# kikimo/tla-raft

Measured on AMD Instinct MI355X. Metric: distinct states/sec (whole node) + wall-time to exhaust, higher is better.
Workload: dtype u32

## Files before the change

tla-raft_amd/csrc/rmc_engine.hip:

```cpp
#include <hip/hip_runtime.h>
#include <hipcub/hipcub.hpp>

#include <algorithm>
#include <array>
#include <chrono>
#include <condition_variable>
#include <cstdio>
#include <cstdlib>
#include <cstring>
#include <memory>
#include <mutex>
#include <string>
#include <thread>
#include <vector>

#include <fcntl.h>
#include <sys/mman.h>
#include <unistd.h>

#include "rmc.h"
#include "rmc_kernels.h"
#include "rmc_plan.h"
#include "rmc_spec.h"

// ... 448 lines not shown
    std::vector<TraceStep> trace;
    double seconds = 0;

    KParams base(const Shard &s) const {
        KParams P{};
        P.d = U.d;
        P.E = cfg.max_election;
        P.R = cfg.max_restart;
        P.seeded = cfg.spec_variant == RMC_SPEC_SEEDED;
        P.quirks = (cfg.spec_variant == RMC_SPEC_SPLIT_BRAIN ? 1u : 0u) | (cfg.spec_variant == RMC_SPEC_COMMIT_PAST_LOG ? 2u : 0u);
        P.check_deadlock = cfg.check_deadlock;
        P.inv_mask = cfg.invariants;
        P.inv_order = inv_order;
        P.t.info = d_info;
        P.t.nat2id = d_nat2id;
        P.t.gmsg = d_gmsg;
        P.t.seeds = d_seeds;
        P.t.np = np;
        P.t.bmw = (uint32_t)((U.info.size() + 31) / 32);
        P.seen = s.seen();
        P.rcap = ~0ull;
        P.err = s.err;
        P.flags = s.flags;
        P.par = s.par;
        P.pslot = s.pslot;
        P.trace_base = s.tdev;
        return P;
    }

    void ring_params(const Shard &s, KParams &P) const {
        P.front = s.R;
        P.foff = s.cur_off;
        P.fbase = s.cur_wbase;
        P.rcap = s.rcap;
        P.next = s.R;
        P.noff = s.nxt_off;
        P.nbase = s.nbase();
    }

    KParams chunk_params(const Shard &s) const {
        KParams Q = base(s);
        ring_params(s, Q);
        Q.cnt = s.cnt; Q.fp = s.fp; Q.wpos = s.wpos; Q.wcnt = s.wcnt; Q.wacc = s.wacc; Q.pnm = s.pnm;
        Q.wposw = s.wposw; Q.bw = s.bw; Q.bg = s.bg; Q.boff = s.boff; Q.bww = s.bww; Q.boffw = s.boffw;
        Q.bn = s.bn; Q.boffn = s.boffn;
        Q.tickets = s.tickets; Q.ctick = s.ctick; Q.sum = s.sum;
        Q.score = s.score; Q.lslot = s.lslot; Q.ET = s.E; Q.hctx = s.hctx;
        return Q;
    }

    const int lookahead = env_int("RMC_LOOKAHEAD", 1, 0, 1);
    bool two_sets() const { return lookahead && !multi; }

    void swap_staging(Shard &s) {
        Staging &a = s.alt;
        std::swap(s.score, a.score); std::swap(s.hctx, a.hctx); std::swap(s.cnt, a.cnt); std::swap(s.pnm, a.pnm);
        std::swap(s.hcnt, a.hcnt); std::swap(s.hoff, a.hoff);
        std::swap(s.err, a.err); std::swap(s.sum, a.sum); std::swap(s.flags, a.flags);
        std::swap(s.xdone, a.done); std::swap(s.xt0, a.t0); std::swap(s.xt1, a.t1); std::swap(s.xtimed, a.timed);
        s.ocnt = reinterpret_cast<uint32_t *>(s.sum + SUM_OCNT);
    }
    static void alt_params(const Staging &a, KParams &Q) {
        Q.score = a.score; Q.hctx = a.hctx; Q.cnt = a.cnt; Q.pnm = a.pnm;
        Q.err = a.err; Q.sum = a.sum; Q.flags = a.flags;
    }
    void xwait() {
        if (xpending) HIPCHK(hipStreamSynchronize(xstream));
    }
    void drop_lookahead() {
        if (!xpending) return;
        xpending = false;
        (void)hipStreamSynchronize(xstream);
        Shard &s = sh[0];
        (void)hipMemsetAsync(s.alt.err, 0xFF, ERR_NSLOTS * 8, xstream);
        (void)hipMemsetAsync(s.alt.flags, 0, 16, xstream);
        (void)hipMemsetAsync(s.alt.sum, 0, SUM_WORDS_TOTAL * 8, xstream);
        (void)hipStreamSynchronize(xstream);
    }
    struct XDrain {
        rmc_ctx *c;
        ~XDrain() { c->drop_lookahead(); }
    };

    void pack(const int32_t *u, uint32_t *rec) const {
        const int n = N, Vv = V;
        std::vector<uint32_t> w(Layout<MAXN, MAXV>::NW + 8, 0);
        int k = 0;
        auto L_VF = 0, L_CT = 1, L_ROLE = 2, L_CI = 3, L_LL = 4, L_LOG = 5, L_MI = 5 + n, L_NI = 5 + 2 * n,
             L_PEND = 5 + 3 * n, L_MISC = 6 + 3 * n;
        auto check = [](int v, int lo, int hi, const char *what) {
            if (v < lo || v > hi) throw Fail(RMC_E_ARG, std::string("state field out of range: ") + what);
        };
        for (int i = 0; i < n; i++) {
            check(u[k + i], -1, n - 1, "votedFor");
            w[L_VF] = setnib(w[L_VF], i, u[k + i] < 0 ? VF_NONE : (uint32_t)u[k + i]);
        }
        k += n;
        for (int i = 0; i < n; i++) { check(u[k + i], 0, 7, "currentTerm"); w[L_CT] = setnib(w[L_CT], i, u[k + i]); }
        k += n;
        for (int i = 0; i < n; i++) { check(u[k + i], 0, 2, "role"); w[L_ROLE] = setnib(w[L_ROLE], i, u[k + i]); }
        k += n;
        for (int i = 0; i < n; i++) { check(u[k + i], 1, Vv + 1, "commitIndex"); w[L_CI] = setnib(w[L_CI], i, u[k + i]); }
        k += n;
        std::vector<int> ll(n);
        for (int i = 0; i < n; i++) {
            check(u[k + i], 1, Vv + 1, "Len(logs)");
// ... 1152 lines not shown
            for (Shard &t : sh) fix_ring(t, sh.size());
        replicated = false;
    }
    uint64_t *old_off_ = nullptr;
    int pending_fail = 0;
    std::string pending_msg;

    std::string flag_msg(unsigned long long f) const {
        if (f & 1u) return "a state exceeds msg_cap = " + std::to_string(ks.MCAP) + " messages";
        if (f & 2u) return "internal: a split chunk's parent records are not consecutive in the frontier ring";
        if (f & 4u) return "race probe: the commit's arrival counters were not all re-armed when the level finished";
        return "internal: unknown flag " + std::to_string(f);
    }
    static int flag_code(unsigned long long f) { return (f & 1u) ? RMC_E_CAPACITY : RMC_E_STATE; }

    static int first_error(const unsigned long long *e, unsigned long long *best) {
        int kind = -1;
        *best = ~0ull;
        const int order[4] = {ERR_ASSERT, ERR_DEADLOCK, ERR_INV, ERR_EVAL};
        for (int q = 0; q < 4; q++) {
            const int kk = order[q];
            if (e[kk] == ~0ull) continue;
            if (kind < 0 || (e[kk] >> 8) < (*best >> 8)) { kind = kk; *best = e[kk]; }
        }
        return kind;
    }

    void renew_election_tags(Shard &s, uint32_t ahead) {
        if (!s.E || s.epoch + ahead - s.lxy_epoch0 < 0xFFFFu) return;
        launch_eslot_clear(s.E, s.lcap, stream);
        s.lxy_epoch0 = s.epoch;
    }

    void end_level(Shard &s, uint64_t gid_nxt, int L) {
        std::swap(s.cur_off, s.nxt_off);
        std::swap(s.cur_off_cap, s.nxt_off_cap);
        s.cur_wbase = s.nbase();
        s.cur_words = s.nxt_words;
        s.nxt_words = 0;
        s.cur_n = s.nxt_n;
        s.nxt_n = 0;
        if (s.cur_n) s.level_start.push_back(gid_nxt);
        (void)L;
    }

    int step_single(rmc_level_stats *st) {
        auto t0 = std::chrono::steady_clock::now();
        Shard &s = sh[0];
        const int L = (int)s.level_start.size();
        st->level = L;
        st->expanded = s.cur_n;
        const uint64_t gid_cur = s.level_start[L - 1];
        const uint64_t gid_nxt = gid_cur + s.cur_n;
        uint64_t level_gen = 0, level_self = 0;
        s.nxt_n = 0;
        s.nxt_words = 0;
        const uint64_t MSW = (uint64_t)ks.maxsucc * (uint64_t)ks.RECW_MAX;
        XDrain drain{this};
        bool ahead = false;
        const bool time_hash = timing_on && (!cfg.timing_phases || (cfg.timing_phases & (1u << PH_HASH)));
        for (uint64_t p0 = 0; p0 < s.cur_n; p0 += chunk_parents) {
            const uint64_t p1 = std::min(s.cur_n, p0 + chunk_parents), np_ = p1 - p0;
            const bool expanded = ahead;
            ahead = false;
            if (expanded) {
                swap_staging(s);
                HIPCHK(hipStreamWaitEvent(stream, s.xdone, 0));
                xpending = false;
                if (s.xtimed) evrecs.push_back({PH_HASH, s.xt0, s.xt1});
            }
            const uint64_t Gub = np_ * (uint64_t)ks.maxsucc;
            maybe_migrate(s, s.T_count + Gub);
            const bool may_small = Gub <= (1ull << 20);
            uint64_t consumed = (s.ring_fixed && p0 && may_small) ? d2h(s.cur_off + p0) : 0;
            const bool small = may_small && seen_room(s, s.T_count + Gub) && ring_room(s, np_ * MSW, consumed);
            if (small) {
                ensure_ring(s, np_ * MSW, consumed);
                ensure_off(s.nxt_off, s.nxt_off_cap, s.nxt_n, s.nxt_n + Gub);
                grow_trace(s, Gub);
                grow_seen(s, s.T_count + Gub);
            }
            ensure_chunk(s, Gub);
            const uint64_t Lcap = std::min(next_pow2(2 * Gub), s.lcap);
            renew_election_tags(s, 1);
            ++s.epoch;
            trace_restart(s);
            const bool split = split_min && np_ >= split_min;
            const bool fold = split && ks.maxsucc <= 256;
            auto params = [&] {
                KParams Q = chunk_params(s);
                Q.p_begin = p0; Q.p_end = p1; Q.next_base = s.nxt_n; Q.next_wbase = s.nxt_words;
                Q.gid_next_base = gid_nxt; Q.gid_parent_base = gid_cur;
                Q.Lmask = Lcap - 1;
                Q.epoch = s.epoch;
                Q.split = split ? (fold ? 1 : 7) : 0;
                Q.plist = split ? s.plist : nullptr;
                Q.hcnt = split ? s.hcnt : nullptr;
                Q.hoff = fold ? s.hoff : nullptr;
                s.chunk_sep = Q.hcnt != nullptr;
                s.chunk_dense = Q.hoff != nullptr;
                return Q;
            };
            constexpr size_t SUM_CLEAR = (SUM_SELF_STRIPE + SELF_STRIDE * SELF_STRIPES - SUM_SELF) * 8;
            if (!expanded) {
                HIPCHK(hipMemsetAsync(s.sum + SUM_SELF, 0, SUM_CLEAR, stream));
                timed(PH_HASH, [&] {
                    if (split) ks.split(params(), stream);
                    else ks.fused(params(), stream);
                });
            }
            auto look_ahead = [&] {
                const uint64_t q1 = std::min(s.cur_n, p1 + chunk_parents);
                if (!two_sets() || !split || p1 >= s.cur_n || q1 - p1 < split_min || s.gslots < Gcap ||
                    !s.alt.score || !s.alt.hctx)
                    return;
                KParams Q = params();
                alt_params(s.alt, Q);
                Q.p_begin = p1;
                Q.p_end = q1;
                Q.hcnt = s.alt.hcnt;
                Q.hoff = fold ? s.alt.hoff : nullptr;
                xpending = true;
                HIPCHK(hipMemsetAsync(s.alt.sum + SUM_SELF, 0, SUM_CLEAR, xstream));
                s.alt.timed = time_hash;
                if (time_hash) HIPCHK(hipEventRecord(s.alt.t0, xstream));
                ks.split(Q, xstream);
                if (time_hash) HIPCHK(hipEventRecord(s.alt.t1, xstream));
                HIPCHK(hipEventRecord(s.alt.done, xstream));
                ahead = true;
            };
            look_ahead();
            if (split) timed(PH_OTHER, [&] { ks.hash_probe(params(), np_, stream); });
            timed(PH_DEDUP, [&] {
                ks.wincount(params(), np_, stream);
                if (split) launch_nzlist(params(), np_, stream);
            });
            if (!small) {
                HIPCHK(hipMemcpyAsync(s.hsum, s.sum, 8 * 8, hipMemcpyDeviceToHost, stream));
                unsigned long long *hc = s.hsum + SUM_WORDS_TOTAL - 1;
                const bool read_consumed = s.ring_fixed && p0 && !may_small;
                if (read_consumed) HIPCHK(hipMemcpyAsync(hc, s.cur_off + p0, 8, hipMemcpyDeviceToHost, stream));
                HIPCHK(hipStreamSynchronize(stream));
                if (read_consumed) consumed = *hc;
                collect_times(st);
                const uint64_t Wub = s.hsum[1], Wwords = s.hsum[SUM_WORDS];
                ensure_ring(s, Wwords, consumed);
                ensure_off(s.nxt_off, s.nxt_off_cap, s.nxt_n, s.nxt_n + Wub);
                grow_trace(s, Wub);
                grow_seen(s, s.T_count + Wub);
            }
            trace_fence(s);
            if (split && !fold) timed(PH_DEDUP, [&] { ks.insert(params(), np_, stream); });
            timed(PH_MAT, [&] {
                if (split) ks.commit_split(params(), np_, stream);
                else ks.commit(params(), stream);
            });
            HIPCHK(hipMemcpyAsync(s.hsum, s.sum, (SUM_SELF + 1) * 8, hipMemcpyDeviceToHost, stream));
            HIPCHK(hipStreamSynchronize(stream));
            HIPCHK(hipGetLastError());
            collect_times(st);
            const uint64_t G = s.hsum[0], Wn = s.hsum[1], Ww = s.hsum[SUM_WORDS];
            level_self += s.hsum[SUM_SELF];
            if (s.hsum[2 + ERR_NSLOTS]) throw Fail(flag_code(s.hsum[2 + ERR_NSLOTS]), flag_msg(s.hsum[2 + ERR_NSLOTS]));
            flush_trace(s, gid_nxt + s.nxt_n + Wn);
            level_gen += G;
            s.T_count += Wn;
            unsigned long long best;
            const int kind = first_error(s.hsum + 2, &best);
            if (kind >= 0) {
                drop_lookahead();
                stop_on_error(kind, best, p0, s.nxt_n, gid_cur, gid_nxt, level_gen - G, st);
                st->seconds = std::chrono::duration<double>(std::chrono::steady_clock::now() - t0).count();
                seconds += st->seconds;
                return status;
            }
            s.nxt_n += Wn;
            s.nxt_words += Ww;
            s.peak_words = std::max(s.peak_words, s.cur_words - consumed + s.nxt_words);
        }
        total_generated += level_gen;
        total_distinct += s.nxt_n;
        st->generated = level_gen;
        st->self_loops = level_self;
        st->new_states = s.nxt_n;
        st->new_bytes = s.nxt_words * 4;
        end_level(s, gid_nxt, L);
        if (s.cur_n) {
            depth = L + 1;
        } else {
            finished = true;
            status = RMC_DONE;
            queue_at_end = 0;
        }
        HIPCHK(hipStreamSynchronize(stream));
        st->total_generated = total_generated;
        st->total_distinct = total_distinct;
        st->queue = s.cur_n;
        st->status = finished ? RMC_DONE : RMC_OK;
        st->seconds = std::chrono::duration<double>(std::chrono::steady_clock::now() - t0).count();
        seconds += st->seconds;
        return st->status;
    }

    static int env_int(const char *name, int dflt, int lo, int hi) {
        const char *v = std::getenv(name);
        if (!v || !*v) return dflt;
        return std::max(lo, std::min(hi, std::atoi(v)));
    }
    const uint64_t split_min = (uint64_t)env_int("RMC_SPLIT_MIN", 1 << 16, 0, 1 << 30);
    const int dl_group = env_int("RMC_DL_GROUP", 2, 1, 64);
    const int dl_ahead = env_int("RMC_DL_AHEAD", 2, 1, 64);
    const int dl_query_us = env_int("RMC_DL_QUERY_US", 2000, 0, 1 << 30);
    int batch_levels() const { return cfg.device_levels ? (int)cfg.device_levels : LREC_CAP; }
    uint64_t dev_parents() const { return std::min<uint64_t>(chunk_parents, 1ull << 15); }
    bool batch_ok() const {
        const Shard &s = sh[0];
        const uint64_t first = s.cur_n * (uint64_t)ks.maxsucc;
        return (!multi || (replicated && s.cur_n < shard_min)) && inited && !finished && cfg.device_levels != 1 &&
               s.cur_n > 0 && s.cur_n <= dev_parents() && ring_room(s, first * (uint64_t)ks.RECW_MAX, 0) &&
               seen_room(s, s.T_count + 2 * first);
    }

    int step_batch(rmc_level_stats *out, int maxl) {
        auto t0 = std::chrono::steady_clock::now();
        Shard &s = sh[0];
        const uint64_t DP = dev_parents(), MS = (uint64_t)ks.maxsucc;
        const int K = std::max(1, std::min(maxl, LREC_CAP));
        uint64_t target = std::min(std::max<uint64_t>(s.cur_n * MS * 32, 1ull << 16), DP * MS);
        maybe_migrate(s, s.T_count + 2 * target);
        if (!ring_room(s, s.cur_n * MS * (uint64_t)ks.RECW_MAX, 0) || !seen_room(s, s.T_count + 2 * s.cur_n * MS))
            return 0;
        if (s.ring_fixed) target = std::min<uint64_t>(target, (s.rcap - s.cur_words) / (uint64_t)ks.RECW_MAX);
        if (s.Tc) target = std::min<uint64_t>(target, ((uint64_t)(0.9 * (double)s.T_cap) - s.T_count) / 2);
        target = std::max<uint64_t>(target, s.cur_n * MS);
        s.nxt_words = 0;
        ensure_ring(s, target * (uint64_t)ks.RECW_MAX, 0);
// ... 1632 lines not shown
```

tla-raft_amd/csrc/rmc_kernels.h:

```cpp
#pragma once
#include <hip/hip_runtime.h>
#include <stdint.h>

#include "rmc_spec.h"

namespace rmc {

struct Tables {
    const uint32_t *info;
    const uint16_t *nat2id;
    const ulonglong2 *gmsg;
    const uint64_t *seeds;
    int np;
    uint32_t bmw;
};

struct ESlot {
    unsigned long long x, y;
    unsigned long long k;
    unsigned long long pad;
};

struct Seen {
    ulonglong2 *T;
    unsigned long long *Tc;
    uint64_t mask;
    uint64_t cap;
};

enum ErrSlot { ERR_ASSERT = 0, ERR_DEADLOCK = 1, ERR_INV = 2, ERR_EVAL = 3, ERR_NSLOTS = 4 };

enum CtlStop : uint32_t { CTL_RUN = 0, CTL_DONE = 1, CTL_ERROR = 2, CTL_HOST = 3 };
struct LevelCtl {
    unsigned long long cur_n;
    unsigned long long gid_cur;
    unsigned long long T_count;
    unsigned long long Lmask;
    unsigned long long cur_wbase, cur_words;
    unsigned long long off_cap, rcap, trace_base, trace_cap, T_cap, chunk_parents, Lcap_max;
    uint32_t level;
    uint32_t epoch;
    uint32_t stop;
    uint32_t done_levels;
    uint32_t batch;
    uint32_t pad_;
};
struct LevelRec { unsigned long long expanded, generated, new_states, words, self_loops; };
constexpr int LREC_CAP = 1024;
struct HostLoop {
    uint32_t done;
    uint32_t stop;
    uint32_t pad_[2];
    LevelCtl ctl;
    LevelRec rec[LREC_CAP];
};
constexpr uint32_t WTILE = 1024;
constexpr uint32_t WTILES_MAX = 4096;
constexpr int SUM_WORDS = 7;
constexpr int SUM_INS = 9;
constexpr int SUM_INS_COMMIT = 10;
constexpr int SUM_NZ = 16;
constexpr int SUM_SELF = 17;
constexpr int SUM_HFP = 18;
constexpr int SUM_OCNT = 20;
constexpr int SUM_SELF_STRIPE = 64, SELF_STRIDE = 16, SELF_STRIPES = 8;
constexpr int SUM_WORDS_TOTAL = 192;


struct KParams {
    Dims d;
    int E, R, seeded, check_deadlock;
    uint32_t inv_mask;
    uint32_t inv_order;
    Tables t;
    const uint32_t *front;
    const uint64_t *foff;
    uint64_t fbase, rcap;
    uint64_t p_begin, p_end;
    uint32_t *cnt;
    uint32_t *hcnt;
    uint32_t *hoff;
    const uint32_t *off;
    ulonglong2 *fp;
    const uint32_t *wflag;
    uint32_t *wpos;
    Seen seen;
    uint32_t *next;
    uint64_t *noff;
    uint64_t nbase;
    uint64_t next_wbase;
    uint64_t next_base;
    uint64_t *par;
    uint16_t *pslot;
    uint64_t trace_base;
    uint64_t gid_next_base;
    uint64_t gid_parent_base;
    unsigned long long *err;
    uint32_t *flags;
    int route;
    uint4 *xside;
    uint32_t *ocnt;
    uint32_t nown;
    ESlot *OT;
    uint64_t ot_mask, gblk;
    uint32_t ot_round, self;
    int split;
    uint32_t *hctx;
    uint32_t quirks;
    uint4 *score;
    uint32_t *lslot;
    ESlot *ET;
    uint64_t Lmask;
    uint32_t epoch;
    uint32_t *wcnt;
    uint32_t *wacc;
    uint32_t *pnm;
    uint32_t *wposw;
    uint32_t *bw, *bg, *boff;
    uint32_t *bww, *boffw;
    uint32_t *bn, *boffn;
    uint32_t *plist;
    uint32_t *tickets;
    uint32_t *ctick;
    unsigned long long *sum;
    LevelCtl *ctl;
    LevelCtl *ctl_next;
    LevelRec *lrec;
    HostLoop *hloop;
    uint32_t done_levels;
    uint32_t *out_keys;
    uint32_t *out_count;
};

struct KernelSet {
    int N, V, MR, MCAP, CCW, RECW_MAX, maxsucc;
    int ctxw;
    void (*single)(const KParams &, hipStream_t);
    void (*fused)(const KParams &, hipStream_t);
    void (*split)(const KParams &, hipStream_t);
    void (*hash_probe)(const KParams &, uint64_t np, hipStream_t);
    void (*insert)(const KParams &, uint64_t np, hipStream_t);
    void (*wincount)(const KParams &, uint64_t np, hipStream_t);
    void (*commit)(const KParams &, hipStream_t);
    void (*commit_split)(const KParams &, uint64_t np, hipStream_t);
    void (*local_elect)(const KParams &, uint64_t np, Seen, ESlot *OT, uint64_t mask,
                        uint32_t round, uint32_t W, uint32_t self, uint64_t g0, hipStream_t);
    void (*local_flags)(const KParams &, uint64_t np, Seen, const ESlot *OT, uint32_t round, uint32_t W,
                        uint32_t self, uint64_t g0, unsigned long long *inserted, hipStream_t);
    void (*fp_states)(const KParams &, uint64_t n, hipStream_t);
    void (*inv_states)(const KParams &, uint64_t n, int32_t *out, hipStream_t);
    void (*encode)(const uint32_t *nibble_core, uint32_t *packed);
    void (*decode)(const uint32_t *packed, uint32_t *nibble_core);
};

bool get_kernels(int N, int V, int msg_cap, bool become_follower, KernelSet *ks);

constexpr uint32_t LS_SEEN = 0xFFFFFFFFu, LS_ELECT = 0xFFFFFFFEu, LS_WIN = 0xFFFFFFFDu;
void launch_rehash(const ulonglong2 *Told, uint64_t old_cap, Seen dst, hipStream_t s);
void launch_eslot_clear(ESlot *t, uint64_t n, hipStream_t s);
void launch_insert_fps(const ulonglong2 *fp, uint64_t n, Seen seen, hipStream_t s);
// ... 26 lines not shown
```

tla-raft_amd/csrc/rmc_kernels.hip:

```cpp
#include <hip/hip_runtime.h>


#include "rmc_kernels.h"

#ifdef RMC_PHASE_PROF
__device__ unsigned long long g_phase[16];
#define PHASE_DECL unsigned long long _acc[8] = {0, 0, 0, 0, 0, 0, 0, 0}; long long _tp = clock64();
#define PHASE(k) do { const long long _t = clock64(); _acc[k] += (unsigned long long)(_t - _tp); _tp = _t; } while (0)
#define PHASE_FLUSH_AT(b) do { if (threadIdx.x == 0) for (int _k = 0; _k < 8; _k++) atomicAdd(&g_phase[(b) + _k], _acc[_k]); } while (0)
#define PHASE_FLUSH PHASE_FLUSH_AT(0)
extern "C" int rmc_debug_phases(unsigned long long *out, int reset) {
    if (hipMemcpyFromSymbol(out, HIP_SYMBOL(g_phase), sizeof(unsigned long long) * 16) != hipSuccess) return -1;
    if (reset) {
        unsigned long long z[16] = {0};
        if (hipMemcpyToSymbol(HIP_SYMBOL(g_phase), z, sizeof(z)) != hipSuccess) return -1;
    }
    return 16;
}
#else
#define PHASE_DECL
#define PHASE(k) do {} while (0)
#define PHASE_FLUSH do {} while (0)
#define PHASE_FLUSH_AT(b) do {} while (0)
#endif
// ... 1029 lines not shown
    e[0] = a0.x; e[1] = a0.y; e[2] = a1.x; e[3] = a1.y; e[4] = a2.x; e[5] = a2.y; e[6] = a3.x; e[7] = a3.y;
}

__device__ __forceinline__ bool seen_contains(const Seen &S, ulonglong2 f) {
    if (S.Tc) {
        const uint64_t nbk = S.cap / TB;
        uint64_t b = t_home_c(f, nbk);
        for (;;) {
            unsigned long long e[TB];
            bucket_load(S.Tc, b, e);
            bool hit = false, free_ = false;
#pragma unroll
            for (uint64_t k = 0; k < TB; k++) {
                hit |= e[k] == f.x;
                free_ |= e[k] == 0ull;
            }
            if (hit) return true;
            if (free_) return false;
            b = (b + 1 == nbk) ? 0 : b + 1;
        }
    }
    uint64_t h = t_index(f, S.mask);
    for (;;) {
        const ulonglong2 e = S.T[h];
        asm volatile("" ::"v"(e.x), "v"(e.y));
        if (e.x == 0ull) return false;
        if (e.x == f.x && e.y == f.y) return true;
        h = (h + 1) & S.mask;
    }
}

__device__ __forceinline__ void seen_insert(const Seen &S, ulonglong2 f) {
    if (S.Tc) {
        const uint64_t nbk = S.cap / TB;
        uint64_t b = t_home_c(f, nbk);
        for (;;) {
            unsigned long long e[TB];
            bucket_load(S.Tc, b, e);
            for (uint64_t k = 0; k < TB; k++)
                if (e[k] == 0ull && atomicCAS(&S.Tc[b * TB + k], 0ull, (unsigned long long)f.x) == 0ull) return;
            b = (b + 1 == nbk) ? 0 : b + 1;
        }
    }
    uint64_t h = t_index(f, S.mask);
    for (;;) {
        unsigned long long prev = atomicCAS((unsigned long long *)&S.T[h].x, 0ull, (unsigned long long)f.x);
        if (prev == 0ull) { S.T[h].y = f.y; return; }
        h = (h + 1) & S.mask;
    }
}

__device__ __forceinline__ uint64_t l_index(const ulonglong2 f, uint64_t mask) {
    return (f.x ^ (f.x >> 31) ^ (f.y >> 7)) & mask;
}
__device__ __forceinline__ uint32_t fp_owner(const ulonglong2 f, uint32_t W) {
    return (uint32_t)((f.y >> 40) % W);
}

__device__ __forceinline__ uint32_t elect_tag(uint32_t epoch) { return epoch % 0xFFFFu + 1u; }
__device__ __forceinline__ unsigned long long elect_key(uint32_t epoch, uint64_t q, uint32_t e) {
    return ((unsigned long long)(0xFFFFFFFFu - epoch) << 32) | ((unsigned long long)(uint32_t)q << 2) | e;
}
__device__ __forceinline__ uint32_t elect_q(unsigned long long w) { return (uint32_t)w >> 2; }

template <int MAXS>
__device__ __forceinline__ uint32_t elect_slot(ESlot *E, uint32_t *wacc, uint64_t mask,
                                               uint32_t epoch, const ulonglong2 f, uint64_t q, uint32_t e, uint64_t g,
                                               unsigned long long v) {
    const unsigned long long tag = elect_tag(epoch);
    const unsigned long long xk = (f.x & ~0xFFFFull) | tag, yk = (f.y & ~0xFFFFull) | tag;
    for (;;) {
        unsigned long long *px = &E[g].x, *py = &E[g].y;
        if ((v & 0xFFFFull) != tag) {
            const unsigned long long prev = atomicCAS(px, v, xk);
            if (prev == v) {
#ifdef RMC_RACE_PROBE
                if ((q & 7u) == 0u) race_delay(2);
#endif
                __hip_atomic_store(py, yk, __ATOMIC_RELAXED, __HIP_MEMORY_SCOPE_AGENT);
                break;
            }
            v = prev;
            if ((v & 0xFFFFull) != tag) continue;
        }
        if (v == xk) {
            const unsigned long long y = __hip_atomic_load(py, __ATOMIC_RELAXED, __HIP_MEMORY_SCOPE_AGENT);
            if ((y & 0xFFFFull) != tag) {
                v = __hip_atomic_load(px, __ATOMIC_RELAXED, __HIP_MEMORY_SCOPE_AGENT);
                continue;
            }
            if (y == yk) break;
        }
        g = (g + 1) & mask;
        v = __hip_atomic_load(&E[g].x, __ATOMIC_RELAXED, __HIP_MEMORY_SCOPE_AGENT);
    }
    const unsigned long long mine = elect_key(epoch, q, e);
    const unsigned long long old = atomicMin(&E[g].k, mine);
    if (old > mine) {
        atomicAdd(&wacc[q / MAXS], 1u + (e << 12));
        if ((old >> 32) == (mine >> 32)) atomicSub(&wacc[elect_q(old) / MAXS], 1u + ((uint32_t)(old & 3u) << 12));
    }
    return (uint32_t)g;
}

template <int N, int V, int MR>
__device__ __forceinline__ void stage_succ(const Succ<N, V, MR> &o, uint32_t nm, uint4 *dst) {
// ... 991 lines not shown
            }
            if (tid < IC_N) sCc[tid] = 0u;
            __syncthreads();
            PHASE(6);
            if ((uint32_t)tid < nI) {
                const uint32_t kb = (sItm[j] - ibase) * NCI, cn = sCnt[j];
                const uint64_t pl = b0 + j;
                const uint64_t q0 = (!FUSE && P.hoff) ? (uint64_t)sHo[j] : pl * (uint64_t)MX;
#pragma unroll
                for (int c = 0; c < NCI; c++) {
                    const RowSucc<S::NADD> &x = c ? ob : o;
                    if (x.key == KEY_NONE || (!FUSE && x.self && P.hcnt)) continue;
                    uint32_t rank = 0;
                    for (uint32_t e = 0; e < cn; e++) rank += (uint32_t)sKey[kb + e] < x.key ? 1u : 0u;
                    const uint64_t q = q0 + rank;
                    if constexpr (FUSE) {
                        if (x.self) {
                            P.lslot[q] = LS_SEEN;
                            atomicAdd(&sSelfN, 1u);
                            continue;
                        }
                        uint4 st4[S::SW4];
                        row_stage<S::NADD>(x, nmj, S::SW4, st4);
                        uint4 *dst = P.score + q * (uint64_t)S::SW4;
#pragma unroll
                        for (int w = 0; w < S::SW4; w++) dst[w] = st4[w];
                        const unsigned long long *m0 = sM0 + j * NPR, *m1 = sM1 + j * NPR;
                        const ulonglong2 f = staged_fp<N, V, MR>(
                            P, sCore + j * NWP, [&](int pi) { return make_ulonglong2(m0[pi], m1[pi]); },
                            [&](int a, uint32_t) { return x.ainf[a]; }, st4[0], st4[1],
                            S::SW4 > 2 ? st4[S::SW4 > 2 ? 2 : 0] : make_uint4(0u, 0u, 0u, 0u), sK);
                        P.fp[q] = f;
                        P.lslot[q] = probe_elect<MX>(P, f, q, (x.nadd + (nmj & 1u) + 1u) >> 1, P.Lmask);
                    } else {
                        row_stage<S::NADD>(x, nmj, S::SW4, P.score + q * (uint64_t)S::SW4);
                    }
                }
            }
            PHASE(5);
            a = b;
        }
    }
    __syncthreads();
    if constexpr (FUSE) {
        if (tid == 0 && sSelfN)
            atomicAdd(&P.sum[SUM_SELF_STRIPE + SELF_STRIDE * (blockIdx.x % SELF_STRIPES)], (unsigned long long)sSelfN);
    } else {
        if (tid == 0 && sHfp) atomicAdd(&P.sum[SUM_HFP], (unsigned long long)sHfp);
    }
    PHASE_FLUSH;
}

template <int MX, class F>
__device__ __forceinline__ void each_successor(const KParams &P, F &&f) {
    const int lane = threadIdx.x & 63;
    const uint64_t np = P.p_end - P.p_begin;
    const uint64_t nwaves = (uint64_t)gridDim.x * (blockDim.x >> 6);
    for (uint64_t g0 = ((uint64_t)blockIdx.x * (blockDim.x >> 6) + (threadIdx.x >> 6)) * 64; g0 < np;
         g0 += nwaves * 64) {
        const uint64_t pl = g0 + (uint64_t)lane;
        const uint32_t t = pl < np ? (P.hcnt ? P.hcnt : P.cnt)[pl] : 0u;
        const uint32_t h0 = (pl < np && P.hoff) ? P.hoff[pl] : 0u;
        uint32_t tot;
        const uint32_t ex = wave_excl_scan(t, lane, &tot);
        for (uint32_t b0 = 0; b0 < tot; b0 += 64) {
            const uint32_t i = b0 + (uint32_t)lane;
            int j = 0;
#pragma unroll
            for (int st = 32; st; st >>= 1) {
                const uint32_t v = (uint32_t)__shfl(ex, j + st, 64);
                j = v <= i ? j + st : j;
            }
            const uint32_t exj = (uint32_t)__shfl(ex, j, 64);
            const uint32_t hj = (uint32_t)__shfl(h0, j, 64);
            const uint64_t pj = g0 + (uint64_t)j;
            if (i < tot) f(pj, i - exj, P.hoff ? (uint64_t)hj + (i - exj) : pj * (uint64_t)MX + (i - exj));
        }
    }
}

__device__ __forceinline__ unsigned long long owner_key(uint32_t tag, uint64_t key) {
    return ((unsigned long long)(0xFFFFu - tag) << 48) | key;
}
__device__ __forceinline__ uint64_t owner_order(uint64_t gparent, uint32_t rank, uint32_t e) {
    return (((gparent << 10) | rank) << 2) | e;
}
__device__ __forceinline__ bool owner_same(unsigned long long k, unsigned long long want) { return (k | 3ull) == (want | 3ull); }
struct OwnerLocal {
    uint32_t *wacc;
    uint64_t g0, np;
};
__device__ __forceinline__ uint32_t owner_bid(ESlot *OT, uint64_t mask, uint32_t tag32,
                                              const ulonglong2 f, uint64_t key, const OwnerLocal &loc) {
    const unsigned long long tag = tag32;
    const unsigned long long xk = (f.x & ~0xFFFFull) | tag, yk = (f.y & ~0xFFFFull) | tag;
    uint64_t g = l_index(f, mask);
    unsigned long long v = __hip_atomic_load(&OT[g].x, __ATOMIC_RELAXED, __HIP_MEMORY_SCOPE_AGENT);
    bool done = false;
    while (!done) {
        bool next = false;
        if ((v & 0xFFFFull) != tag) {
            const unsigned long long prev = atomicCAS(&OT[g].x, v, xk);
            if (prev == v) {
#ifdef RMC_RACE_PROBE
                if ((key & 7u) == 0u) race_delay(2);
#endif
                __hip_atomic_store(&OT[g].y, yk, __ATOMIC_RELAXED, __HIP_MEMORY_SCOPE_AGENT);
                done = true;
            } else {
                v = prev;
            }
        }
        if (!done && (v & 0xFFFFull) == tag) {
            if (v == xk) {
                const unsigned long long y = __hip_atomic_load(&OT[g].y, __ATOMIC_RELAXED, __HIP_MEMORY_SCOPE_AGENT);
                if (y == yk) done = true;
                else if ((y & 0xFFFFull) == tag) next = true;
                else v = __hip_atomic_load(&OT[g].x, __ATOMIC_RELAXED, __HIP_MEMORY_SCOPE_AGENT);
            } else {
                next = true;
            }
        }
        if (next) {
            g = (g + 1) & mask;
            v = __hip_atomic_load(&OT[g].x, __ATOMIC_RELAXED, __HIP_MEMORY_SCOPE_AGENT);
        }
    }
    const unsigned long long nk = owner_key(tag32, key);
    const unsigned long long old = atomicMin(&OT[g].k, nk);
    if (loc.wacc && nk < old) {
        const uint64_t gp = key >> 12;
        if (gp - loc.g0 < loc.np) atomicAdd(&loc.wacc[gp - loc.g0], 1u + ((uint32_t)(key & 3u) << 12));
        if ((old >> 48) == (unsigned long long)(0xFFFFu - tag32)) {
            const uint64_t ok = old & ((1ull << 48) - 1ull), op = ok >> 12;
            if (op - loc.g0 < loc.np) atomicSub(&loc.wacc[op - loc.g0], 1u + ((uint32_t)(ok & 3u) << 12));
        }
    }
    return (uint32_t)g;
}

#ifndef RMC_PROBE_WAVES
#define RMC_PROBE_WAVES 0
#endif
template <int N, int V, int MR, int MX>
__global__ __launch_bounds__(256, RMC_PROBE_WAVES) void k_hash_probe(KParams P) {
    using S = Spec<N, V, MR>;
    using Lo = Layout<N, V>;
    constexpr int CTXW = ctx_words<N, V>(), CC4 = (S::CCW + 3) / 4;
    __shared__ uint64_t sK[2][N * N];
    __shared__ uint32_t sOwn[64];
    if (threadIdx.x < 2 * N * N) {
        const int f = threadIdx.x / (N * N), a = (threadIdx.x / N) % N, b = threadIdx.x % N;
        sK[f][a * N + b] = P.t.seeds[f * SEEDS_PER_F + a * MAXN + b];
    }
    if (threadIdx.x < 64) sOwn[threadIdx.x] = 0u;
    uint64_t Lmask = P.Lmask;
    if (!P.route) {
        const unsigned long long nf = __hip_atomic_load(&P.sum[SUM_HFP], __ATOMIC_RELAXED, __HIP_MEMORY_SCOPE_AGENT);
        const uint64_t want = nf < 512ull ? 1024ull : 1ull << (64 - __clzll((long long)(2 * nf - 1)));
        Lmask = want - 1 < Lmask ? want - 1 : Lmask;
    }
    __syncthreads();
    each_successor<MX>(P, [&](uint64_t pl, uint32_t r, uint64_t sq) {
        const uint64_t q = pl * (uint64_t)MX + r;
        const uint4 *cx = reinterpret_cast<const uint4 *>(P.hctx + pl * (uint64_t)CTXW);
        const uint4 *st = P.score + sq * (uint64_t)S::SW4;
        const uint4 sa = st[0], sb = st[1];
        const uint4 sc = S::SW4 > 2 ? st[2] : make_uint4(0u, 0u, 0u, 0u);
        uint32_t pk[CC4 * 4];
#pragma unroll
        for (int k = 0; k < CC4; k++) {
            const uint4 v = cx[k];
            pk[4 * k] = v.x; pk[4 * k + 1] = v.y; pk[4 * k + 2] = v.z; pk[4 * k + 3] = v.w;
        }
        uint4 mp[N * (N - 1)];
#pragma unroll
        for (int k = 0; k < N * (N - 1); k++) mp[k] = cx[CC4 + k];
        uint32_t pc[Lo::NW];
        decode_core<N, V>(pk, pc);
        const ulonglong2 f = staged_fp<N, V, MR>(P, pc, [&](int pi) {
            const uint4 m = mp[pi];
            return make_ulonglong2((uint64_t)m.y << 32 | m.x, (uint64_t)m.w << 32 | m.z);
        }, [&](int, uint32_t id) { return P.t.info[id]; }, sa, sb, sc, sK);
        const uint32_t nadd = sb.z >> 16;
        P.fp[sq] = f;
        if (P.route) {
            const uint32_t o = fp_owner(f, P.nown);
            if (P.ocnt) atomicAdd(&sOwn[o], 1u);
            if (P.OT) {
                const uint32_t nm = (pc[Lo::W_MISC] >> 16) & 0xFFu;
                P.lslot[sq] = o != P.self ? LS_ELECT
                              : seen_contains(P.seen, f)
                                  ? LS_SEEN
                                  : owner_bid(P.OT, P.ot_mask, P.ot_round + 1u, f,
                                              owner_order(P.gblk + pl, r, (nadd + (nm & 1u) + 1u) >> 1),
                                              OwnerLocal{P.wacc, P.gblk, P.p_end - P.p_begin});
            }
            return;
        }
        const uint32_t nm = (pc[Lo::W_MISC] >> 16) & 0xFFu;
        P.lslot[sq] = probe_elect<MX>(P, f, q, (nadd + (nm & 1u) + 1u) >> 1, Lmask);
    });
    if (P.route && P.ocnt) {
        __syncthreads();
        if (threadIdx.x < P.nown && sOwn[threadIdx.x]) atomicAdd(&P.ocnt[threadIdx.x], sOwn[threadIdx.x]);
    }
}

template <int MX>
__global__ __launch_bounds__(256) void k_insert_winners(KParams P) {
    each_successor<MX>(P, [&](uint64_t pl, uint32_t r, uint64_t sq) {
        const uint64_t q = pl * (uint64_t)MX + r;
        const uint32_t g = P.lslot[sq];
        if (g >= LS_ELECT) return;
        const bool w = elect_q(P.ET[g].k) == (uint32_t)q;
        if (w) seen_insert(P.seen, P.fp[sq]);
        if (P.split & 4) P.lslot[sq] = w ? LS_WIN : LS_SEEN;
    });
}

template <int N, int V, int MR>
__global__ __launch_bounds__(64) void k_fp_states(KParams P, uint64_t n) {
    using S = Spec<N, V, MR>;
    __shared__ uint64_t M0[N * N], M1[N * N];
    __shared__ uint32_t pcore[Layout<N, V>::NW + N];
    const int lane = threadIdx.x;
    for (uint64_t p = blockIdx.x; p < n; p += gridDim.x) {
        Wave<N, V, MR> W;
        load_parent<N, V, MR, true>(P, rec_start<S::RECW_MAX>(P, p), lane, W, M0, M1, pcore);
        const ulonglong2 f = fingerprint<N, V>(W.c, M0, M1, P.t);
        if (lane == 0) P.fp[p] = f;
    }
}

template <int N, int V, int MR>
__global__ __launch_bounds__(64) void k_inv_states(KParams P, uint64_t n, int32_t *out) {
    using S = Spec<N, V, MR>;
    using Lo = Layout<N, V>;
    const uint64_t i = (uint64_t)blockIdx.x * 64 + threadIdx.x;
    if (i >= n) return;
    const uint64_t start = rec_start<S::RECW_MAX>(P, i);
    uint32_t packed[S::CCW], c[Lo::NW];
#pragma unroll
    for (int k = 0; k < S::CCW; k++) packed[k] = ring_word(P.front, start, (uint32_t)k, P.rcap);
    decode_core<N, V>(packed, c);
    const MsgView mv{P.front, ring_wrap(start + S::CCW, P.rcap), P.rcap, (c[Lo::W_MISC] >> 16) & 0xFFu, 0u, 0u, 0u,
                     P.t.info};
    for (int b = 0; b < 7; b++) out[i * 7 + b] = inv_eval<N, V>(c, b, mv);
}

__device__ __forceinline__ uint32_t block_excl_scan(uint32_t v, uint32_t *ws, uint32_t *total) {
    const uint32_t tid = threadIdx.x, lane = tid & 63, wv = tid >> 6;
    uint32_t x = v;
#pragma unroll
    for (int d = 1; d < 64; d <<= 1) {
// ... 844 lines not shown
        }
        const uint32_t nadd = P.score[q * (uint64_t)SW4 + 1].z >> 16;
        P.lslot[q] = owner_bid(OT, mask, round + 1u, f, owner_order(g0 + pl, r, (nadd + (P.pnm[pl] & 1u) + 1u) >> 1), loc);
    });
}

template <int MX>
__global__ __launch_bounds__(256) void k_local_flags(KParams P, Seen seen, const ESlot *OT, uint32_t round,
                                                     uint32_t W, uint32_t self, uint64_t g0,
                                                     unsigned long long *inserted) {
    const uint32_t tag = round + 1u;
    uint32_t mine = 0;
    each_successor<MX>(P, [&](uint64_t pl, uint32_t r, uint64_t q) {
        const uint32_t g = P.lslot[q];
        if (g == LS_ELECT || g == LS_SEEN) return;
        const bool w = owner_same(OT[g].k, owner_key(tag, owner_order(g0 + pl, r, 0u)));
        P.lslot[q] = w ? LS_WIN : LS_SEEN;
        if (w) {
            seen_insert(seen, P.fp[q]);
            mine++;
        }
    });
    block_count_add(mine, inserted);
}

static inline unsigned grid_for(uint64_t n) {
    const uint64_t cap = 256ull * RMC_GRID_PER_CU;
    return (unsigned)(n < cap ? (n ? n : 1) : cap);
}

template <int N, int V, int MR, bool BFV = false>
struct Launch {
    static constexpr int MX = Spec<N, V, MR>::MAXS + (BFV ? Spec<N, V, MR>::MCAP : 0);
    static size_t bm_bytes(const KParams &P) { return (size_t)P.t.bmw * 4; }
    static void single(const KParams &P, hipStream_t s) {
        hipLaunchKernelGGL((k_expand<N, V, MR, M_SINGLE, BFV>), dim3(1), dim3(64), bm_bytes(P), s, P);
    }
    static void fused(const KParams &P, hipStream_t s) {
        if (!P.route) {
            const uint64_t nbat = (P.p_end - P.p_begin + XF_PARENTS - 1) / XF_PARENTS;
            hipLaunchKernelGGL((k_expand_items<N, V, MR, BFV, true, XF_PARENTS>), dim3((unsigned)(nbat < 8192 ? (nbat ? nbat : 1) : 8192)),
                               dim3(XB_THREADS), 0, s, P);
            return;
        }
        hipLaunchKernelGGL((k_expand<N, V, MR, M_FUSED, BFV>), dim3(grid_for(P.p_end - P.p_begin)), dim3(64),
                           bm_bytes(P), s, P);
    }
    static void split(const KParams &P, hipStream_t s) {
        const uint64_t nbat = (P.p_end - P.p_begin + XB_PARENTS - 1) / XB_PARENTS;
        hipLaunchKernelGGL((k_expand_items<N, V, MR, BFV, false, XB_PARENTS>), dim3((unsigned)(nbat < 2048 ? (nbat ? nbat : 1) : 2048)),
                           dim3(items_threads<N, V, MR, false>()), 0, s, P);
    }
    static void hash_probe(const KParams &P, uint64_t np, hipStream_t s) {
        const uint64_t blocks = (np + 255) / 256;
        hipLaunchKernelGGL((k_hash_probe<N, V, MR, MX>), dim3(blocks ? (unsigned)(blocks < 16384ull ? blocks : 16384ull) : 1u),
                           dim3(256), 0, s, P);
    }
    static void insert(const KParams &P, uint64_t np, hipStream_t s) {
        const uint64_t blocks = (np + 255) / 256;
        hipLaunchKernelGGL((k_insert_winners<MX>), dim3(blocks ? (unsigned)(blocks < 16384ull ? blocks : 16384ull) : 1u),
                           dim3(256), 0, s, P);
    }
    static void wincount(const KParams &P, uint64_t np, hipStream_t s) {
        const uint64_t tiles = (np + WTILE - 1) / WTILE;
        hipLaunchKernelGGL((k_wincount<N, V, MR>), dim3(tiles ? (unsigned)tiles : 1u), dim3(1024), 0, s, P);
    }
    static void commit(const KParams &P, hipStream_t s) {
        if constexpr (MX <= XB_THREADS) {
            if (!P.route && !P.split && !P.plist) {
                const uint64_t nbat = (P.p_end - P.p_begin + XC_PARENTS - 1) / XC_PARENTS;
                hipLaunchKernelGGL((k_commit_items<N, V, MR, MX, true, XC_PARENTS>),
                                   dim3((unsigned)(nbat < 8192 ? (nbat ? nbat : 1) : 8192)), dim3(XB_THREADS), 0, s, P);
                return;
            }
        }
        hipLaunchKernelGGL((k_commit<N, V, MR, BFV>), dim3(grid_for(P.p_end - P.p_begin)), dim3(64), 0, s, P);
    }
    static void commit_split(const KParams &P, uint64_t np, hipStream_t s) {
        const uint64_t blocks = (np + 255) / 256;
        if constexpr (MX <= XB_THREADS) {
            {
                const uint64_t nbat = (np + 63) / 64;
                hipLaunchKernelGGL((k_commit_items<N, V, MR, MX, false, 64>), dim3((unsigned)(nbat < 2048 ? (nbat ? nbat : 1) : 2048)),
                                   dim3(XB_THREADS), 0, s, P);
                hipLaunchKernelGGL((k_commit_finish<MX, Spec<N, V, MR>::RECW_MAX>), dim3(1), dim3(64), 0, s, P);
                return;
            }
        }
        hipLaunchKernelGGL((k_commit_split<N, V, MR, MX>), dim3(blocks ? (unsigned)(blocks < 16384ull ? blocks : 16384ull) : 1u),
                           dim3(256), 0, s, P);
        hipLaunchKernelGGL((k_commit_finish<MX, Spec<N, V, MR>::RECW_MAX>), dim3(1), dim3(64), 0, s, P);
    }
    static void local_elect(const KParams &P, uint64_t np, Seen seen, ESlot *OT,
                            uint64_t mask, uint32_t round, uint32_t W, uint32_t self, uint64_t g0, hipStream_t s) {
        const uint64_t blocks = (np + 255) / 256;
        hipLaunchKernelGGL((k_local_elect<MX, Spec<N, V, MR>::SW4>), dim3(blocks ? (unsigned)(blocks < 16384ull ? blocks : 16384ull) : 1u),
                           dim3(256), 0, s, P, seen, OT, mask, round, W, self, g0);
    }
    static void local_flags(const KParams &P, uint64_t np, Seen seen, const ESlot *OT, uint32_t round,
                            uint32_t W, uint32_t self, uint64_t g0, unsigned long long *inserted, hipStream_t s) {
        const uint64_t blocks = (np + 255) / 256;
        hipLaunchKernelGGL((k_local_flags<MX>),
                           dim3(blocks ? (unsigned)(blocks < 16384ull ? blocks : 16384ull) : 1u), dim3(256), 0, s, P,
                           seen, OT, round, W, self, g0, inserted);
    }
    static void fps(const KParams &P, uint64_t n, hipStream_t s) {
        hipLaunchKernelGGL((k_fp_states<N, V, MR>), dim3(grid_for(n)), dim3(64), 0, s, P, n);
    }
    static void invs(const KParams &P, uint64_t n, int32_t *out, hipStream_t s) {
// ... 278 lines not shown
```

Baseline: 963.4 million.

## Add per-wave LDS duplicate filter in hash probe and batch wave runs

Adds a small per-wavefront shared-memory table in the hash probe kernel that catches duplicate fingerprints within a wave's recent successors and marks them seen before the global probe/elect step. This avoids redundant global hash-table traffic for local duplicates. Each wave now also processes several consecutive 64-parent groups (a run), and the grid is shrunk to match, so the table sees more locality. The cost is LDS usage (512 entries per wave), CAS/fence overhead per successor, and fewer blocks, which could reduce occupancy.

```diff
diff --git a/tla-raft_amd/csrc/rmc_engine.hip b/tla-raft_amd/csrc/rmc_engine.hip
--- a/tla-raft_amd/csrc/rmc_engine.hip
+++ b/tla-raft_amd/csrc/rmc_engine.hip
@@ -524,6 +524,17 @@
     const int lookahead = env_int("RMC_LOOKAHEAD", 1, 0, 1);
     bool two_sets() const { return lookahead && !multi; }
 
+    static uint32_t probe_dedup_entries() {
+        const int v = env_int("RMC_PROBE_DEDUP", 1, 0, (int)PD_ENTRIES);
+        if (v <= 1) return v ? PD_ENTRIES : 0u;
+        uint32_t n = 2;
+        while (2 * n <= (uint32_t)v) n *= 2;
+        return n;
+    }
+    const uint32_t probe_dedup = probe_dedup_entries();
+    const uint32_t probe_run = (uint32_t)env_int("RMC_PROBE_RUN", 0, 0, 64);
+    const int probe_log = env_int("RMC_PROBE_DEDUP_LOG", 0, 0, 1);
+
     void swap_staging(Shard &s) {
         Staging &a = s.alt;
         std::swap(s.score, a.score); std::swap(s.hctx, a.hctx); std::swap(s.cnt, a.cnt); std::swap(s.pnm, a.pnm);
@@ -1782,7 +1793,7 @@
         st->expanded = s.cur_n;
         const uint64_t gid_cur = s.level_start[L - 1];
         const uint64_t gid_nxt = gid_cur + s.cur_n;
-        uint64_t level_gen = 0, level_self = 0;
+        uint64_t level_gen = 0, level_self = 0, level_hfp = 0, level_drop = 0;
         s.nxt_n = 0;
         s.nxt_words = 0;
         const uint64_t MSW = (uint64_t)ks.maxsucc * (uint64_t)ks.RECW_MAX;
@@ -1827,6 +1838,8 @@
                 Q.plist = split ? s.plist : nullptr;
                 Q.hcnt = split ? s.hcnt : nullptr;
                 Q.hoff = fold ? s.hoff : nullptr;
+                Q.pdedup = split ? probe_dedup : 0u;
+                Q.prun = probe_run;
                 s.chunk_sep = Q.hcnt != nullptr;
                 s.chunk_dense = Q.hoff != nullptr;
                 return Q;
@@ -1885,12 +1898,16 @@
                 if (split) ks.commit_split(params(), np_, stream);
                 else ks.commit(params(), stream);
             });
-            HIPCHK(hipMemcpyAsync(s.hsum, s.sum, (SUM_SELF + 1) * 8, hipMemcpyDeviceToHost, stream));
+            HIPCHK(hipMemcpyAsync(s.hsum, s.sum, (SUM_PDROP + 1) * 8, hipMemcpyDeviceToHost, stream));
             HIPCHK(hipStreamSynchronize(stream));
             HIPCHK(hipGetLastError());
             collect_times(st);
             const uint64_t G = s.hsum[0], Wn = s.hsum[1], Ww = s.hsum[SUM_WORDS];
             level_self += s.hsum[SUM_SELF];
+            if (split) {
+                level_hfp += s.hsum[SUM_HFP];
+                level_drop += s.hsum[SUM_PDROP];
+            }
             if (s.hsum[2 + ERR_NSLOTS]) throw Fail(flag_code(s.hsum[2 + ERR_NSLOTS]), flag_msg(s.hsum[2 + ERR_NSLOTS]));
             flush_trace(s, gid_nxt + s.nxt_n + Wn);
             level_gen += G;
@@ -1912,6 +1929,9 @@
         total_distinct += s.nxt_n;
         st->generated = level_gen;
         st->self_loops = level_self;
+        if (probe_log)
+            std::fprintf(stderr, "rmc probe_dedup: level %d fingerprinted %llu dropped %llu\n", L,
+                         (unsigned long long)level_hfp, (unsigned long long)level_drop);
         st->new_states = s.nxt_n;
         st->new_bytes = s.nxt_words * 4;
         end_level(s, gid_nxt, L);
diff --git a/tla-raft_amd/csrc/rmc_kernels.h b/tla-raft_amd/csrc/rmc_kernels.h
--- a/tla-raft_amd/csrc/rmc_kernels.h
+++ b/tla-raft_amd/csrc/rmc_kernels.h
@@ -62,7 +62,10 @@
 constexpr int SUM_NZ = 16;
 constexpr int SUM_SELF = 17;
 constexpr int SUM_HFP = 18;
+constexpr uint32_t PD_ENTRIES = 512;
+constexpr int PROBE_RUN = 2;
 constexpr int SUM_OCNT = 20;
+constexpr int SUM_PDROP = 56;
 constexpr int SUM_SELF_STRIPE = 64, SELF_STRIDE = 16, SELF_STRIPES = 8;
 constexpr int SUM_WORDS_TOTAL = 192;
 
@@ -106,6 +109,7 @@
     uint32_t ot_round, self;
     int split;
     uint32_t *hctx;
+    uint32_t pdedup, prun;
     uint32_t quirks;
     uint4 *score;
     uint32_t *lslot;
diff --git a/tla-raft_amd/csrc/rmc_kernels.hip b/tla-raft_amd/csrc/rmc_kernels.hip
--- a/tla-raft_amd/csrc/rmc_kernels.hip
+++ b/tla-raft_amd/csrc/rmc_kernels.hip
@@ -1105,6 +1105,9 @@
 
 __device__ __forceinline__ uint64_t l_index(const ulonglong2 f, uint64_t mask) {
     return (f.x ^ (f.x >> 31) ^ (f.y >> 7)) & mask;
+}
+__device__ __forceinline__ uint32_t pd_index(const ulonglong2 f) {
+    return (uint32_t)(f.x >> 17) ^ (uint32_t)(f.y >> 43);
 }
 __device__ __forceinline__ uint32_t fp_owner(const ulonglong2 f, uint32_t W) {
     return (uint32_t)((f.y >> 40) % W);
@@ -2202,12 +2205,15 @@
 }
 
 template <int MX, class F>
-__device__ __forceinline__ void each_successor(const KParams &P, F &&f) {
+__device__ __forceinline__ void each_successor(const KParams &P, F &&f, uint32_t run = 1) {
     const int lane = threadIdx.x & 63;
     const uint64_t np = P.p_end - P.p_begin;
     const uint64_t nwaves = (uint64_t)gridDim.x * (blockDim.x >> 6);
-    for (uint64_t g0 = ((uint64_t)blockIdx.x * (blockDim.x >> 6) + (threadIdx.x >> 6)) * 64; g0 < np;
-         g0 += nwaves * 64) {
+    const uint64_t span = (uint64_t)run * 64;
+    const uint32_t wv = __builtin_amdgcn_readfirstlane(threadIdx.x >> 6);
+    for (uint64_t r0 = ((uint64_t)blockIdx.x * (blockDim.x >> 6) + wv) * span; r0 < np;
+         r0 += nwaves * span)
+    for (uint64_t g0 = r0; g0 < r0 + span && g0 < np; g0 += 64) {
         const uint64_t pl = g0 + (uint64_t)lane;
         const uint32_t t = pl < np ? (P.hcnt ? P.hcnt : P.cnt)[pl] : 0u;
         const uint32_t h0 = (pl < np && P.hoff) ? P.hoff[pl] : 0u;
@@ -2304,6 +2310,16 @@
         sK[f][a * N + b] = P.t.seeds[f * SEEDS_PER_F + a * MAXN + b];
     }
     if (threadIdx.x < 64) sOwn[threadIdx.x] = 0u;
+    __shared__ ulonglong2 sTab[4 * PD_ENTRIES];
+    __shared__ uint32_t sDrop;
+    const int lane = threadIdx.x & 63;
+    const uint32_t pdN = P.route ? 0u : P.pdedup;
+    const uint32_t tab0 = __builtin_amdgcn_readfirstlane(threadIdx.x >> 6) * PD_ENTRIES;
+    uint32_t ndrop = 0;
+    if (pdN) {
+        for (uint32_t k = (uint32_t)lane; k < pdN; k += 64) sTab[tab0 + k] = make_ulonglong2(0ull, 0ull);
+        if (threadIdx.x == 0) sDrop = 0u;
+    }
     uint64_t Lmask = P.Lmask;
     if (!P.route) {
         const unsigned long long nf = __hip_atomic_load(&P.sum[SUM_HFP], __ATOMIC_RELAXED, __HIP_MEMORY_SCOPE_AGENT);
@@ -2348,9 +2364,44 @@
             }
             return;
         }
+        if (pdN) {
+            unsigned long long *ex = &sTab[tab0 + (pd_index(f) & (pdN - 1u))].x, *ey = ex + 1;
+            const unsigned long long ox = __hip_atomic_load(ex, __ATOMIC_RELAXED, __HIP_MEMORY_SCOPE_WAVEFRONT);
+            const unsigned long long oy = __hip_atomic_load(ey, __ATOMIC_RELAXED, __HIP_MEMORY_SCOPE_WAVEFRONT);
+            bool drop = ox == f.x && oy == f.y;
+            __builtin_amdgcn_fence(__ATOMIC_ACQ_REL, "wavefront");
+            if (!drop) {
+                unsigned long long cur = ox;
+                const unsigned long long claim = (q + 1ull) << 1;
+                const bool won = __hip_atomic_compare_exchange_strong(ex, &cur, claim, __ATOMIC_RELAXED, __ATOMIC_RELAXED,
+                                                                      __HIP_MEMORY_SCOPE_WAVEFRONT);
+                __builtin_amdgcn_fence(__ATOMIC_ACQ_REL, "wavefront");
+                if (won) {
+                    __hip_atomic_store(ey, f.y, __ATOMIC_RELAXED, __HIP_MEMORY_SCOPE_WAVEFRONT);
+                    __hip_atomic_store(ex, f.x, __ATOMIC_RELAXED, __HIP_MEMORY_SCOPE_WAVEFRONT);
+                }
+                __builtin_amdgcn_fence(__ATOMIC_ACQ_REL, "wavefront");
+                __builtin_amdgcn_wave_barrier();
+                if (!won && !(cur & 1ull) && cur < claim) {
+                    const unsigned long long nx = __hip_atomic_load(ex, __ATOMIC_RELAXED, __HIP_MEMORY_SCOPE_WAVEFRONT);
+                    const unsigned long long ny = __hip_atomic_load(ey, __ATOMIC_RELAXED, __HIP_MEMORY_SCOPE_WAVEFRONT);
+                    drop = nx == f.x && ny == f.y;
+                }
+            }
+            ndrop += (uint32_t)__popcll(__ballot(drop));
+            if (drop) {
+                P.lslot[sq] = LS_SEEN;
+                return;
+            }
+        }
         const uint32_t nm = (pc[Lo::W_MISC] >> 16) & 0xFFu;
         P.lslot[sq] = probe_elect<MX>(P, f, q, (nadd + (nm & 1u) + 1u) >> 1, Lmask);
-    });
+    }, P.prun);
+    if (pdN) {
+        if (lane == 0 && ndrop) atomicAdd(&sDrop, ndrop);
+        __syncthreads();
+        if (threadIdx.x == 0 && sDrop) atomicAdd(&P.sum[SUM_PDROP], (unsigned long long)sDrop);
+    }
     if (P.route && P.ocnt) {
         __syncthreads();
         if (threadIdx.x < P.nown && sOwn[threadIdx.x]) atomicAdd(&P.ocnt[threadIdx.x], sOwn[threadIdx.x]);
@@ -3301,9 +3352,13 @@
                            dim3(items_threads<N, V, MR, false>()), 0, s, P);
     }
     static void hash_probe(const KParams &P, uint64_t np, hipStream_t s) {
-        const uint64_t blocks = (np + 255) / 256;
+        KParams Q = P;
+        const uint64_t fit = np / (256ull * 1024ull);
+        Q.prun = P.route ? 1u : P.prun ? P.prun : (uint32_t)(fit < 1 ? 1 : fit < (uint64_t)PROBE_RUN ? fit : (uint64_t)PROBE_RUN);
+        const uint64_t per = 256ull * Q.prun;
+        const uint64_t blocks = (np + per - 1) / per;
         hipLaunchKernelGGL((k_hash_probe<N, V, MR, MX>), dim3(blocks ? (unsigned)(blocks < 16384ull ? blocks : 16384ull) : 1u),
-                           dim3(256), 0, s, P);
+                           dim3(256), 0, s, Q);
     }
     static void insert(const KParams &P, uint64_t np, hipStream_t s) {
         const uint64_t blocks = (np + 255) / 256;
```

Measured after the change: 1.030 billion, median of 6. +6.9%, better.
